# RchalYang/torchrl

Measured on AMD Instinct MI355X. Metric: env_steps_per_sec_ppo_2048env_halfcheetah_shape, higher is better.
Workload: dtype f32

## Files before the change

### torchrl_amd/csrc/k_ppo.hip

```cpp
#include <cstdlib>
#include "trl_common.h"
#include "trl_mlp.h"
#include "trl_head.h"
#include "trl_comm.h"

struct PpoDev {
  const float *obs, *acts, *advs, *rets, *old_values, *old_logp;
  const int64_t* row_idx;
  int rows_mb, N;
  const double* adv_raw;
  double n_global;
  const float *pf_params, *vf_params;
  float clip_para, entropy_coeff;
  int clipped_value_loss, tanh_action;
  int loss_mode;
  float* partial;
  double* scal_partial;
  int n_wg, n_pf, p_stride;
  int D, A;
};

template <int D, int H, int A> struct PpoShape {
  static_assert(H == 64 && D > 16 && D <= 32 && A <= 8, "instantiated for 16 < D <= 32, H == 64, A <= 8");
  static constexpr int P_PF = MlpFlat<D, H, A>::P_PF, P_VF = MlpFlat<D, H, 1>::P_VF;
  static constexpr int P_STRIDE = ((P_PF > P_VF ? P_PF : P_VF) + 63) & ~63;
};

#define WV_WAVES 4
#ifdef TRL_EXP_CLK
#define WCLK_DECL long long clk_prev = clock64(); float clk_acc[24]; for (int q_ = 0; q_ < 24; ++q_) clk_acc[q_] = 0.f;
#define WCLK(ph) { __builtin_amdgcn_sched_barrier(0); const long long c_ = clock64(); clk_acc[ph] += (float)(c_ - clk_prev); clk_prev = c_; __builtin_amdgcn_sched_barrier(0); }
#else
#define WCLK_DECL
#define WCLK(ph)
#endif
#define WV_THREADS (64 * WV_WAVES)
#define LDT 20
#define LDW 68

template <int D, int H, int A> struct WvShape {
  static_assert(H == 64 && (D == 17 || D == 32) && A <= 8, "instantiated for D == 17 / 32, H == 64, A <= 8");
  static constexpr int O_W2F = 0, O_W2B = H * LDW, O_B1 = 2 * H * LDW, O_B2 = O_B1 + H, O_SCR = O_B2 + H;
  static constexpr int O_H1 = 0, O_H2 = H * LDT, O_DZ2 = 2 * H * LDT, O_DO = 3 * H * LDT, WSCR = O_DO + 16 * LDT;
  static constexpr int P_STRIDE = PpoShape<D, H, A>::P_STRIDE;
  static constexpr int MAIN = O_SCR + WV_WAVES * WSCR, FOLD = WV_WAVES * P_STRIDE;
  static constexpr int LDS_FLOATS = MAIN > FOLD ? MAIN : FOLD;
};

template <int D, int H, int A> struct WvShapeSD : WvShape<D, H, A> {
  using B = WvShape<D, H, A>;
  static constexpr int P_PF_SD = H * D + H + H * H + H + 2 * A * H + 2 * A, P_VF = MlpFlat<D, H, 1>::P_VF;
  static constexpr int P_STRIDE = ((P_PF_SD > P_VF ? P_PF_SD : P_VF) + 63) & ~63;
  static constexpr int FOLD = WV_WAVES * P_STRIDE;
  static constexpr int LDS_FLOATS = B::MAIN > FOLD ? B::MAIN : FOLD;
};
template <int D, int H, int A, int HEAD> struct WvPick { using T = WvShape<D, H, A>; };
template <int D, int H, int A> struct WvPick<D, H, A, HEAD_SD> { using T = WvShapeSD<D, H, A>; };
#define SD_HALF_LOG_2PI_PLUS_HALF 1.4189385332046727f

__device__ __forceinline__ f32x4 lds4(const float* p) { return *reinterpret_cast<const f32x4*>(p); }
__device__ __forceinline__ float row_sum16(float v) {
  v += __builtin_bit_cast(float, __builtin_amdgcn_update_dpp(0, __builtin_bit_cast(int, v), 0x128, 0xF, 0xF, false));
  v += __builtin_bit_cast(float, __builtin_amdgcn_update_dpp(0, __builtin_bit_cast(int, v), 0x124, 0xF, 0xF, false));
  v += __builtin_bit_cast(float, __builtin_amdgcn_update_dpp(0, __builtin_bit_cast(int, v), 0x122, 0xF, 0xF, false));
  v += __builtin_bit_cast(float, __builtin_amdgcn_update_dpp(0, __builtin_bit_cast(int, v), 0x121, 0xF, 0xF, false));
  return v;
}

template <int D, int H, int A, int ACT, bool IS_PF, bool CONTIG, bool RT, int HEAD = HEAD_GAUSS>
__device__ void ppo_wave_pass(const PpoDev& a, float* lds, int wg_in_net, int n_wg_net) {
  using S = typename WvPick<D, H, A, HEAD>::T;
  constexpr bool WIDE = D > 17,
                 CAT = HEAD == HEAD_CAT, SD = HEAD == HEAD_SD,
                 SDP = SD && IS_PF;
  static_assert(!WIDE || RT, "the wide tile exists as a runtime-dims instantiation only");
  static_assert(!CAT || (IS_PF && RT), "the categorical head is a policy pass of the runtime-dims kernels");
  static_assert(!SD || RT, "the state-dependent-std head belongs to the runtime-dims kernels");
  constexpr int AS = CAT ? 1 : 0;
  const int Dr = RT ? a.D : D;
  const int O = IS_PF ? (RT ? a.A : A) : 1;
  const int OH = SDP ? 2 * O : O;
  const int F_W1 = 0, F_B1 = H * Dr, F_W2 = F_B1 + H, F_B2 = F_W2 + H * H, F_W3 = F_B2 + H, F_B3 = F_W3 + OH * H,
            F_LS = F_B3 + OH, F_END = (CAT || SDP) ? F_LS : F_LS + O;
  auto sd_has = [&](int o) -> bool { return (o & 7) < O; };
  auto sd_row = [&](int o) -> int { return o < 8 ? o : O + (o - 8); };
  const int PS = RT ? a.p_stride : S::P_STRIDE;
  const int tid = threadIdx.x, lane = tid & 63, wave = tid >> 6;
  const int j = lane & 15, g = lane >> 4, i = j;
  const float* gp = IS_PF ? a.pf_params : a.vf_params;
  WCLK_DECL
  float* W2F = lds + S::O_W2F;
  float* W2B = lds + S::O_W2B;
  float* scr = lds + S::O_SCR + wave * S::WSCR;
  float* H1S = scr + S::O_H1;
  float* H2S = scr + S::O_H2;
  float* DZ2S = scr + S::O_DZ2;
  float* DOS = scr + S::O_DO;

  const double adv_s1 = IS_PF ? a.adv_raw[0] : 0.0, adv_s2 = IS_PF ? a.adv_raw[1] : 0.0;
  const int B = a.rows_mb * a.N;
  const int n_tiles = (B + 15) / 16;
  const int tile_stride = n_wg_net * WV_WAVES;

  float xq[5], xtq[4], lq[6];
  float xq2[4], xtq2[4];
  int tile = wg_in_net * WV_WAVES + wave;
  const int tpr = a.N >> 4;
  int p1r = 0, p1c = 0, p2r = 0, p2c = 0, st_r = 0, st_c = 0;
  int64_t ridx1 = 0, ridx2 = 0;
  bool fv[4], fv2[4];
  const bool f16 = !WIDE && (!RT || Dr > 16), jv = !RT || i < Dr, jv2 = WIDE && 16 + i < Dr;
  const unsigned ox16 = (unsigned)(j * Dr + (f16 ? 16 : 0)) * 4u, os = (unsigned)j * 4u;
  unsigned oxq[4], oxt[4], oa_[4], oxq2[4], oxt2[4];
#pragma unroll
  for (int q = 0; q < 4; ++q) {
    fv[q] = !RT || 4 * g + q < Dr;
    fv2[q] = WIDE && 16 + 4 * g + q < Dr;
    oxq[q] = (unsigned)(j * Dr + (fv[q] ? 4 * g + q : 0)) * 4u;
    oxt[q] = (unsigned)((4 * g + q) * Dr + (jv ? i : 0)) * 4u;
    oxq2[q] = (unsigned)(j * Dr + (fv2[q] ? 16 + 4 * g + q : 0)) * 4u;
    oxt2[q] = (unsigned)((4 * g + q) * Dr + (jv2 ? 16 + i : 0)) * 4u;
    if constexpr (SDP) oa_[q] = (unsigned)(j * O + (4 * (g & 1) + q < O ? 4 * (g & 1) + q : 0)) * 4u;
    else oa_[q] = CAT ? (unsigned)j * 4u : (unsigned)(j * O + (4 * g + q < O ? 4 * g + q : 0)) * 4u;
  }
  auto ldb = [](const float* base, unsigned byte_off) -> float {
    return *reinterpret_cast<const float*>(reinterpret_cast<const char*>(base) + byte_off);
  };
  auto pos_advance = [&](int& r, int& c) { c += st_c; r += st_r; if (c >= tpr) { c -= tpr; ++r; } };
  auto load_ridx = [&](int r) -> int64_t {
    const int rr = r < a.rows_mb ? r : 0;
    return a.row_idx ? a.row_idx[rr] : (int64_t)rr;
  };
  auto fetch_contig = [&](int64_t ridx, int r, int c) {
    const int64_t cell0 = (r < a.rows_mb) ? ridx * a.N + 16 * c : 0;
    const float* ob = a.obs + cell0 * Dr;
#pragma unroll
    for (int q = 0; q < 4; ++q) xq[q] = ldb(ob, oxq[q]);
// ... 66 lines not shown
      fetch_inputs(pn, nt * 16);
      fetch_row(nt + tile_stride);
    }
  };
  if constexpr (CONTIG) {
    const int t0 = __builtin_amdgcn_readfirstlane(tile);
    const int ts = __builtin_amdgcn_readfirstlane(tile_stride);
    st_r = ts / tpr; st_c = ts - st_r * tpr;
    int r0 = t0 / tpr, c0 = t0 - (t0 / tpr) * tpr;
    fetch_contig(load_ridx(r0), r0, c0);
    p1r = r0; p1c = c0;
    pos_advance(p1r, p1c);
    ridx1 = load_ridx(p1r);
    p2r = p1r; p2c = p1c;
    pos_advance(p2r, p2c);
    ridx2 = load_ridx(p2r);
  } else {
    fetch_row(tile);
    const int64_t p0 = (tile * 16 + j < B) ? ridx_nn * a.N + e_nn : 0;
    fetch_inputs(p0, tile * 16);
    fetch_row(tile + tile_stride);
  }
  constexpr int NV = H * H / (4 * WV_THREADS);
  f32x4 wv[NV], wt[NV];
  const int tc = tid & 63, tq = tid >> 6;
  const float bias1 = tid < H ? gp[F_B1 + tid] : 0.0f, bias2 = tid < H ? gp[F_B2 + tid] : 0.0f;
  {
    static_assert(WV_THREADS == 256 && H == 64, "the transposed staging maps (column, 4 rows) onto 256 threads");
    const bool w2_al = !RT || ((reinterpret_cast<uintptr_t>(gp + F_W2) & 15) == 0);
#pragma unroll
    for (int t = 0; t < NV; ++t) {
      if (w2_al) wv[t] = *reinterpret_cast<const f32x4*>(gp + F_W2 + 4 * (tid + WV_THREADS * t));
      else {
#pragma unroll
        for (int x = 0; x < 4; ++x) wv[t][x] = gp[F_W2 + 4 * (tid + WV_THREADS * t) + x];
      }
    }
#pragma unroll
    for (int t = 0; t < NV; ++t)
#pragma unroll
      for (int x = 0; x < 4; ++x) wt[t][x] = gp[F_W2 + (4 * (tq + 4 * t) + x) * H + tc];
  }
  for (int e = lane; e < 16 * LDT; e += 64) DOS[e] = 0.0f;
  float w1[4][5], w3h[4][4], w3t[4][4];
  float w1b[4][4];
#pragma unroll
  for (int so = 0; so < 4; ++so) {
    const int row = 16 * so + i;
#pragma unroll
    for (int r = 0; r < 4; ++r) w1[so][r] = fv[r] ? gp[F_W1 + row * Dr + (fv[r] ? 4 * g + r : 0)] : 0.0f;
    w1[so][4] = (g == 0 && f16) ? gp[F_W1 + row * Dr + (f16 ? 16 : 0)] : 0.0f;
    if constexpr (WIDE) {
#pragma unroll
      for (int r = 0; r < 4; ++r) w1b[so][r] = fv2[r] ? gp[F_W1 + row * Dr + (fv2[r] ? 16 + 4 * g + r : 0)] : 0.0f;
    }
#pragma unroll
    for (int r = 0; r < 4; ++r) {
      if constexpr (SDP) {
        const int o = 4 * g + r;
        w3h[so][r] = sd_has(i) ? gp[F_W3 + (sd_has(i) ? sd_row(i) : 0) * H + 16 * so + 4 * g + r] : 0.0f;
        w3t[so][r] = sd_has(o) ? gp[F_W3 + (sd_has(o) ? sd_row(o) : 0) * H + row] : 0.0f;
      } else if constexpr (IS_PF) {
        w3h[so][r] = (i < O) ? gp[F_W3 + (i < O ? i : 0) * H + 16 * so + 4 * g + r] : 0.0f;
        const int o = 4 * g + r;
        w3t[so][r] = (o < O) ? gp[F_W3 + (o < O ? o : 0) * H + row] : 0.0f;
      } else {
        w3h[so][r] = gp[F_W3 + 16 * so + 4 * g + r];
        w3t[so][r] = 0.0f;
      }
    }
  }
  float lsv[4], ivv[4], b3v[4], lspass[4];
#pragma unroll
  for (int r = 0; r < 4; ++r) {
    const int o = 4 * g + r;
    const float raw = (IS_PF && !CAT && !SDP && o < O) ? gp[F_LS + (o < O ? o : 0)] : 0.0f;
    lsv[r] = fminf(fmaxf(raw, -20.0f), 2.0f);
    ivv[r] = __expf(-2.0f * lsv[r]);
    lspass[r] = (raw >= -20.0f && raw <= 2.0f) ? 1.0f : 0.0f;
    if constexpr (SDP) b3v[r] = sd_has(o) ? gp[F_B3 + (sd_has(o) ? sd_row(o) : 0)] : 0.0f;
    else b3v[r] = (o < O) ? gp[F_B3 + (o < O ? o : 0)] : 0.0f;
  }
  const float vb3 = IS_PF ? 0.0f : gp[F_B3];
#pragma unroll
  for (int t = 0; t < NV; ++t) {
    const int e = 4 * (tid + WV_THREADS * t), r = e / H, c = e - r * H;
    *reinterpret_cast<f32x4*>(W2F + r * LDW + c) = wv[t];
    *reinterpret_cast<f32x4*>(W2B + tc * LDW + 4 * (tq + 4 * t)) = wt[t];
  }
  if (tid < H) { lds[S::O_B1 + tid] = bias1; lds[S::O_B2 + tid] = bias2; }
  __syncthreads();

  const double ng = a.n_global;
  const double adv_mean = adv_s1 / ng;
  const double adv_var = (adv_s2 - adv_s1 * adv_s1 / ng) / (ng - 1.0);
  const float adv_mu = (float)adv_mean;
  const float adv_rstd = 1.0f / ((float)sqrt(fmax(adv_var, 0.0)) + 1e-5f);
  const float inv_b = (float)(1.0 / ng);

  f32x4 gW2[4][4], gW1[4], gW3[4];
  f32x4 gW1b[4];
  float gb1[4][4], gb2[4][4], gW1c[4][4];
  float db3[4], dls[4], stv[7];
  float ent_sum = 0.0f;
  float sdst[8] = {0.0f, 0.0f, -INFINITY, -INFINITY, 0.0f, 0.0f, -INFINITY, -INFINITY}, sd_cnt = 0.0f;
#pragma unroll
  for (int x = 0; x < 4; ++x) {
    gW1[x] = gW3[x] = gW1b[x] = f32x4{0.f, 0.f, 0.f, 0.f};
    db3[x] = dls[x] = 0.0f;
#pragma unroll
    for (int y = 0; y < 4; ++y) { gW2[x][y] = f32x4{0.f, 0.f, 0.f, 0.f}; gb1[x][y] = gb2[x][y] = gW1c[x][y] = 0.0f; }
  }
#pragma unroll
  for (int k = 0; k < 7; ++k) stv[k] = (k >= 2 && k <= 5) ? -INFINITY : 0.0f;

  WCLK(0)
  for (; tile < n_tiles; tile += tile_stride) {
    const int s = tile * 16 + j;
    const bool valid = CONTIG ? true : (s < B);
    float xb[5], xt[4], lin[6], xb2[4], xt2[4];
#pragma unroll
    for (int r = 0; r < 4; ++r) xb[r] = (valid && fv[r]) ? xq[r] : 0.0f;
    xb[4] = (valid && f16) ? xq[4] : 0.0f;
#pragma unroll
    for (int q = 0; q < 4; ++q) xt[q] = (jv && (CONTIG || tile * 16 + 4 * g + q < B)) ? xtq[q] : 0.0f;
    if constexpr (WIDE) {
#pragma unroll
      for (int q = 0; q < 4; ++q) {
        xb2[q] = (valid && fv2[q]) ? xq2[q] : 0.0f;
        xt2[q] = (jv2 && (CONTIG || tile * 16 + 4 * g + q < B)) ? xtq2[q] : 0.0f;
      }
    }
#pragma unroll
    for (int q = 0; q < 6; ++q) lin[q] = lq[q];
    const float x16 = xb[4];

#define PIN_DS() __builtin_amdgcn_sched_barrier(0x676)
    f32x4 h1[4], h2[4];
    f32x4 wq[4], bq;
#pragma unroll
    for (int so = 0; so < 4; ++so) h1[so] = lds4(lds + S::O_B1 + 16 * so + 4 * g);
#pragma unroll
    for (int sl = 0; sl < 4; ++sl) wq[sl] = lds4(W2F + i * LDW + 16 * sl + 4 * g);
    bq = lds4(lds + S::O_B2 + 4 * g);
    PIN_DS();
    WCLK(9)
#pragma unroll
    for (int q = 0; q < (WIDE ? 4 : 5); ++q)
#pragma unroll
      for (int so = 0; so < 4; ++so) h1[so] = mfma16(w1[so][q], xb[q], h1[so]);
    if constexpr (WIDE) {
#pragma unroll
      for (int q = 0; q < 4; ++q)
#pragma unroll
        for (int so = 0; so < 4; ++so) h1[so] = mfma16(w1b[so][q], xb2[q], h1[so]);
    }
    WCLK(10)
#pragma unroll
    for (int so = 0; so < 4; ++so)
#pragma unroll
      for (int r = 0; r < 4; ++r) {
        h1[so][r] = act_fn<ACT>(h1[so][r]);
        H1S[(16 * so + 4 * g + r) * LDT + j] = h1[so][r];
      }
    WCLK(1)
#pragma unroll
// ... 202 lines not shown
      }
#pragma unroll
      for (int so = 0; so < 4; ++so)
#pragma unroll
        for (int r = 0; r < 4; ++r) {
          dz2[so][r] = dv * w3h[so][r];
          gW3[so][r] = fmaf(dv, h2[so][r], gW3[so][r]);
        }
    }
#pragma unroll
    for (int so = 0; so < 4; ++so)
#pragma unroll
      for (int r = 0; r < 4; ++r) {
        dz2[so][r] *= act_grad<ACT>(h2[so][r]);
        gb2[so][r] += dz2[so][r];
        DZ2S[(16 * so + 4 * g + r) * LDT + j] = dz2[so][r];
      }

    WCLK(3)
    f32x4 dz1[4];
    f32x4 hb[4], za2;
#pragma unroll
    for (int so = 0; so < 4; ++so) dz1[so] = f32x4{0.f, 0.f, 0.f, 0.f};
#pragma unroll
    for (int sl = 0; sl < 4; ++sl) {
      f32x4 w[4];
#pragma unroll
      for (int so = 0; so < 4; ++so) w[so] = wb[so];
      if (sl < 3) {
#pragma unroll
        for (int so = 0; so < 4; ++so) wb[so] = lds4(W2B + (16 * so + i) * LDW + 16 * (sl + 1) + 4 * g);
      } else {
#pragma unroll
        for (int c = 0; c < 4; ++c) hb[c] = lds4(H1S + (16 * c + j) * LDT + 4 * g);
        za2 = lds4(DZ2S + i * LDT + 4 * g);
      }
      PIN_DS();
#pragma unroll
      for (int r = 0; r < 4; ++r)
#pragma unroll
        for (int so = 0; so < 4; ++so) dz1[so] = mfma16(w[so][r], dz2[sl][r], dz1[so]);
    }
    WCLK(17)
#pragma unroll
    for (int so = 0; so < 4; ++so)
#pragma unroll
      for (int r = 0; r < 4; ++r) {
        dz1[so][r] *= act_grad<ACT>(h1[so][r]);
        gb1[so][r] += dz1[so][r];
        if constexpr (!WIDE) gW1c[so][r] = fmaf(dz1[so][r], x16, gW1c[so][r]);
        H2S[(16 * so + 4 * g + r) * LDT + j] = dz1[so][r];
      }
    f32x4 za1[4];
#pragma unroll
    for (int so = 0; so < 4; ++so) za1[so] = lds4(H2S + (16 * so + i) * LDT + 4 * g);
    PIN_DS();

    WCLK(4)
#pragma unroll
    for (int so = 0; so < 4; ++so) {
      const f32x4 za = za2;
      if (so < 3) { za2 = lds4(DZ2S + (16 * (so + 1) + i) * LDT + 4 * g); PIN_DS(); }
#pragma unroll
      for (int q = 0; q < 4; ++q)
#pragma unroll
        for (int c = 0; c < 4; ++c) gW2[so][c] = mfma16(za[q], hb[c][q], gW2[so][c]);
    }
    WCLK(5)
#pragma unroll
    for (int so = 0; so < 4; ++so)
#pragma unroll
      for (int q = 0; q < 4; ++q) gW1[so] = mfma16(za1[so][q], xt[q], gW1[so]);
    if constexpr (WIDE) {
#pragma unroll
      for (int so = 0; so < 4; ++so)
#pragma unroll
        for (int q = 0; q < 4; ++q) gW1b[so] = mfma16(za1[so][q], xt2[q], gW1b[so]);
    }
#undef PIN_DS
    WCLK(6)
  }

  __syncthreads();
  float* gimg = lds + wave * S::P_STRIDE;
  for (int e = F_END + lane; e < PS; e += 64) gimg[e] = 0.0f;
#pragma unroll
  for (int so = 0; so < 4; ++so)
#pragma unroll
    for (int r = 0; r < 4; ++r) {
      const int f = 16 * so + 4 * g + r;
#pragma unroll
      for (int c = 0; c < 4; ++c) gimg[F_W2 + f * H + 16 * c + j] = gW2[so][c][r];
      if (jv) gimg[F_W1 + f * Dr + j] = gW1[so][r];
      if (WIDE && jv2) gimg[F_W1 + f * Dr + 16 + j] = gW1b[so][r];
      const float c16 = WIDE ? 0.0f : row_sum16(gW1c[so][r]), s1 = row_sum16(gb1[so][r]), s2 = row_sum16(gb2[so][r]);
      if (j == 0) { if (f16) gimg[F_W1 + f * Dr + 16] = c16; gimg[F_B1 + f] = s1; gimg[F_B2 + f] = s2; }
      if constexpr (IS_PF) {
        const int o = 4 * g + r;
        if constexpr (SDP) { if (sd_has(o)) gimg[F_W3 + sd_row(o) * H + 16 * so + j] = gW3[so][r]; }
        else if (o < O) gimg[F_W3 + o * H + 16 * so + j] = gW3[so][r];
      } else {
        const float w3s = row_sum16(gW3[so][r]);
        if (j == 0) gimg[F_W3 + f] = w3s;
      }
    }
#pragma unroll
  for (int r = 0; r < 4; ++r) {
    const int o = 4 * g + r;
    const float b3 = row_sum16(db3[r]), dl = row_sum16(dls[r]);
    if constexpr (SDP) { if (j == 0 && sd_has(o)) gimg[F_B3 + sd_row(o)] = b3; }
    else if (j == 0 && o < O) {
      gimg[F_B3 + o] = b3;
      if (IS_PF && !CAT) gimg[F_LS + o] = dl;
    }
  }
  WCLK(7)
  __syncthreads();
  const int wg = blockIdx.x;
  static_assert(S::P_STRIDE % 4 == 0, "partial rows are folded and stored 16 bytes at a time");
  for (int e4 = tid; e4 < PS / 4; e4 += WV_THREADS) {
    f32x4 acc = lds4(lds + 4 * e4);
#pragma unroll
    for (int w = 1; w < WV_WAVES; ++w) acc += lds4(lds + w * S::P_STRIDE + 4 * e4);
    *reinterpret_cast<f32x4*>(a.partial + (size_t)wg * a.p_stride + 4 * e4) = acc;
  }
  WCLK(8)
#ifdef TRL_EXP_CLK
  if (tid == 0) for (int ph = 0; ph < 24; ++ph) a.partial[(size_t)wg * a.p_stride + PS - 40 + ph] = clk_acc[ph];
#endif
  __syncthreads();
  double* sred = reinterpret_cast<double*>(lds);
  {
    const bool own = g == 0;
    const double v0 = wave_sum(own ? (double)stv[0] : 0.0), v1 = wave_sum(own ? (double)stv[1] : 0.0),
                 v6 = wave_sum(own ? (double)stv[6] : 0.0);
    const float v2 = wave_max(own ? stv[2] : -INFINITY), v3 = wave_max(own ? stv[3] : -INFINITY),
                v4 = wave_max(own ? stv[4] : -INFINITY), v5 = wave_max(own ? stv[5] : -INFINITY);
    double v7 = 0.0;
    if constexpr (CAT || SDP) v7 = wave_sum(own ? (double)ent_sum : 0.0);
    if (lane == 0) {
      double* p = sred + wave * 8;
      p[0] = v0; p[1] = v1; p[2] = v2; p[3] = v3; p[4] = v4; p[5] = v5; p[6] = v6; p[7] = v7;
    }
    if constexpr (SDP) {
      double e[SD_SCAL];
#pragma unroll
      for (int k = 0; k < 8; ++k) e[k] = (k & 2) ? (double)wave_max(sdst[k]) : wave_sum((double)sdst[k]);
      e[8] = wave_sum((double)sd_cnt);
      if (lane == 0) {
#pragma unroll
        for (int k = 0; k < SD_SCAL; ++k) sred[WV_WAVES * 8 + wave * SD_SCAL + k] = k < 9 ? e[k] : 0.0;
      }
    }
  }
  __syncthreads();
  if (tid < 8) {
    double r = sred[tid];
    for (int w = 1; w < WV_WAVES; ++w) {
      const double o = sred[w * 8 + tid];
      r = (tid >= 2 && tid <= 5) ? fmax(r, o) : r + o;
    }
    a.scal_partial[(size_t)wg * 8 + tid] = r;
  }
  if constexpr (SDP) {
    if (tid >= 64 && tid < 64 + SD_SCAL) {
      const int k = tid - 64;
      double r = sred[WV_WAVES * 8 + k];
      for (int w = 1; w < WV_WAVES; ++w) {
        const double o = sred[WV_WAVES * 8 + w * SD_SCAL + k];
        r = (k < 8 && (k & 2)) ? fmax(r, o) : r + o;
      }
      a.scal_partial[(size_t)a.n_wg * 8 + (size_t)wg * SD_SCAL + k] = r;
    }
  }
}

#define RED_CHUNK 64
#ifndef RED_WAVES
#define RED_WAVES 8
#endif
#ifndef RED_DEPTH
#define RED_DEPTH 16
#endif
__device__ __forceinline__ float fold_chain_tree(float (&acc)[RED_DEPTH]) {
#pragma unroll
  for (int st = RED_DEPTH / 2; st > 0; st >>= 1)
#pragma unroll
    for (int k = 0; k < st; ++k) acc[k] += acc[k + st];
  return acc[0];
}
__device__ __forceinline__ float fold_rows_wave(const float* __restrict__ src, int nrow, int p_stride, int w, bool in_range) {
  float acc[RED_DEPTH];
#pragma unroll
  for (int k = 0; k < RED_DEPTH; ++k) acc[k] = 0.0f;
  if (in_range) {
    for (; w < nrow; w += RED_DEPTH * RED_WAVES) {
      float v[RED_DEPTH];
#pragma unroll
      for (int k = 0; k < RED_DEPTH; ++k) v[k] = (w + RED_WAVES * k < nrow) ? src[(size_t)(w + RED_WAVES * k) * p_stride] : 0.0f;
#pragma unroll
      for (int k = 0; k < RED_DEPTH; ++k) acc[k] += v[k];
    }
  }
  return fold_chain_tree(acc);
}
__device__ __forceinline__ float fold_waves_tree(const float (*s_acc)[RED_CHUNK], int lane) {
  float t4[RED_WAVES / 4];
#pragma unroll
  for (int q = 0; q < RED_WAVES / 4; ++q)
    t4[q] = (s_acc[4 * q][lane] + s_acc[4 * q + 1][lane]) + (s_acc[4 * q + 2][lane] + s_acc[4 * q + 3][lane]);
// ... 319 lines not shown
      const float g_ = first ? gval0 : grads[ge];
      const float mo = first ? m_old : a.m[ge], vo = first ? v_old : a.v[ge], po = first ? p_old : a.params[ge];
      const float gr = g_ * a.grad_scale * s_coef[net];
      const float m = a.beta1 * mo + (1.0f - a.beta1) * gr;
      const float v = a.beta2 * vo + (1.0f - a.beta2) * gr * gr;
      a.m[ge] = m; a.v[ge] = v;
      const float denom = sqrtf(v) / bc2_sqrt + a.eps;
      a.params[ge] = po - ((net == 0 ? lr_pf : lr_vf) / bc1) * (m / denom);
    }
  }
}

template <int D, int H, int A, int ACT, bool CONTIG, bool RT, int HEAD = HEAD_GAUSS>
__global__ __launch_bounds__(WV_THREADS, 1) void ppo_grad_wave_kernel(PpoDev a) {
  static_assert(HEAD == HEAD_GAUSS || RT, "categorical / state-dependent-std head: runtime-dims tiles");
  constexpr int HEAD_VF = HEAD == HEAD_CAT ? HEAD_GAUSS : HEAD;
  extern __shared__ __attribute__((aligned(16))) float lds[];
#ifdef TRL_CHAIN_CLK
  const unsigned long long clk0 = wall_clock64();
#endif
  if ((int)blockIdx.x < a.n_pf) ppo_wave_pass<D, H, A, ACT, true, CONTIG, RT, HEAD>(a, lds, blockIdx.x, a.n_pf);
  else                          ppo_wave_pass<D, H, A, ACT, false, CONTIG, RT, HEAD_VF>(a, lds, blockIdx.x - a.n_pf, a.n_wg - a.n_pf);
#ifdef TRL_CHAIN_CLK
  __syncthreads();
  if (threadIdx.x == 0) {
    a.scal_partial[(size_t)blockIdx.x * 8 + 7] = (double)wall_clock64();
    float* pad = a.partial + (size_t)blockIdx.x * a.p_stride + a.p_stride - 3;
    pad[0] = (float)(clk0 >> 40); pad[1] = (float)((clk0 >> 20) & 0xFFFFFull); pad[2] = (float)(clk0 & 0xFFFFFull);
  }
#endif
}

template <int D, int H, int O, int ACT>
__global__ __launch_bounds__(256) void mlp2_forward_kernel(const float* __restrict__ params,
                                                           const float* __restrict__ x,
                                                           float* __restrict__ out, int M) {
  using L = MlpLds<D, H, O>;
  constexpr int NT = H / 32, KS = ksteps_for(D);
  __shared__ __attribute__((aligned(16))) float sp[L::SIZE];
  const int tid = threadIdx.x, lane = tid & 63, wave = tid >> 6, i = lane & 31, hi = lane >> 5;
  L::load(sp, params, false, tid, 256);
  __syncthreads();
  const int n_tiles = (M + 31) / 32;
  for (int tile = blockIdx.x * 4 + wave; tile < n_tiles; tile += gridDim.x * 4) {
    const int s = tile * 32 + i;
    float xb[KS];
#pragma unroll
    for (int q = 0; q < KS; ++q) { const int k = rowmap(q, hi); xb[q] = (k < D && s < M) ? x[(size_t)s * D + k] : 0.0f; }
    f32x16 h1[NT], h2[NT];
#pragma unroll
    for (int mo = 0; mo < NT; ++mo)
      h1[mo] = act_tile<ACT>(layer1_tile<D, L::LD1, KS>(bias_tile(sp + L::B1 + 32 * mo, hi), sp + L::W1, mo, xb, i, hi));
#pragma unroll
    for (int mo = 0; mo < NT; ++mo)
      h2[mo] = act_tile<ACT>(layer_tile<NT, L::LD2>(bias_tile(sp + L::B2 + 32 * mo, hi), sp + L::W2, mo, h1, i, hi));
    float o[O];
    head_fwd<NT, H, O>(sp + L::W3, sp + L::B3, h2, hi, o);
    if (hi == 0 && s < M) {
#pragma unroll
      for (int c = 0; c < O; ++c) out[(size_t)s * O + c] = o[c];
    }
  }
}

#define SHAPE_IS(d, h, o) (D == (d) && H == (h) && A == (o))

static int ppo_stride_for(int D, int H, int A, int head) {
  if (head == HEAD_GAUSS && SHAPE_IS(17, 64, 6)) return PpoShape<17, 64, 6>::P_STRIDE;
  if (head_shape_ok(head, D, H, A)) {
    const int p_pf = ppo_p_pf(D, H, A, head), p_vf = ppo_p_vf(D, H);
    return ((p_pf > p_vf ? p_pf : p_vf) + 63) & ~63;
  }
  trl_set_error("trl_ppo_%spartial_stride: shape D=%d H=%d A=%d not instantiated (H == 64, 2 <= D <= 32, %d <= A <= %d)",
                HEADS[head].tag, D, H, A, HEADS[head].a_min, HEADS[head].a_max);
  return TRL_EUNSUPPORTED;
}
extern "C" int trl_ppo_partial_stride(int D, int H, int A) { return ppo_stride_for(D, H, A, HEAD_GAUSS); }
extern "C" int trl_ppo_cat_partial_stride(int D, int H, int A) { return ppo_stride_for(D, H, A, HEAD_CAT); }
extern "C" int trl_ppo_sd_partial_stride(int D, int H, int A) { return ppo_stride_for(D, H, A, HEAD_SD); }
extern "C" int trl_ppo_cat_supported(int D, int H, int A, int act) { return head_supported(HEAD_CAT, D, H, A, act); }
extern "C" int trl_ppo_sd_supported(int D, int H, int A, int act) { return head_supported(HEAD_SD, D, H, A, act); }
extern "C" int trl_ppo_sd_scalar_stride(void) { return HEADS[HEAD_SD].scal_stride; }
static_assert(WvShapeSD<17, 64, 8>::P_STRIDE == 6400 && WvShapeSD<32, 64, 8>::P_STRIDE == 7360, "SD image strides at A = 8");
static_assert(WvShapeSD<32, 64, 8>::LDS_FLOATS * sizeof(float) <= 160 * 1024, "SD fold images fit the LDS");

template <int D, int H, int A, int ACT, bool CONTIG, bool RT, int HEAD>
static int launch_ppo_v(const PpoDev& d, hipStream_t s) {
  using S = typename WvPick<D, H, A, HEAD>::T;
  const size_t lds = S::LDS_FLOATS * sizeof(float);
  static bool attr_set = false;
  if (!attr_set) {
    hipError_t e = hipFuncSetAttribute((const void*)ppo_grad_wave_kernel<D, H, A, ACT, CONTIG, RT, HEAD>,
                                       hipFuncAttributeMaxDynamicSharedMemorySize, (int)lds);
    if (e != hipSuccess) { trl_set_error("ppo_grad: hipFuncSetAttribute: %s", hipGetErrorString(e)); return (int)e; }
    attr_set = true;
  }
  hipLaunchKernelGGL((ppo_grad_wave_kernel<D, H, A, ACT, CONTIG, RT, HEAD>), dim3(d.n_wg), dim3(WV_THREADS), lds, s, d);
  TRL_LAUNCH_CHECK();
  return TRL_OK;
}
template <int D, int H, int A, int ACT, bool RT, int HEAD = HEAD_GAUSS>
static int launch_ppo(const PpoDev& d, hipStream_t s) {
  return (d.N % 16 == 0) ? launch_ppo_v<D, H, A, ACT, true, RT, HEAD>(d, s) : launch_ppo_v<D, H, A, ACT, false, RT, HEAD>(d, s);
}

extern "C" int trl_ppo_wg_split(int D, int H, int A, int n_tiles, int n_wg) {
  if (n_wg < 2 || n_tiles <= 0) { trl_set_error("trl_ppo_wg_split: need n_wg >= 2 and n_tiles > 0"); return TRL_EINVAL; }
  const double c_pf = 16.7, c_vf = 12.1;
  int best = n_wg / 2;
  double best_t = 1e300;
  for (int x = 1; x < n_wg; ++x) {
    const double t_pf = (double)((n_tiles + WV_WAVES * x - 1) / (WV_WAVES * x)) * c_pf;
    const double t_vf = (double)((n_tiles + WV_WAVES * (n_wg - x) - 1) / (WV_WAVES * (n_wg - x))) * c_vf;
    const double t = t_pf > t_vf ? t_pf : t_vf;
    if (t < best_t - 1e-9 || (t < best_t + 1e-9 && abs(2 * x - n_wg) < abs(2 * best - n_wg))) { best_t = t; best = x; }
  }
  (void)D; (void)H; (void)A;
  return best;
}
static int resolve_pf_wgs(int n_wg, int n_wg_pf) { return n_wg_pf < 0 ? 0 : (n_wg_pf > 0 ? n_wg_pf : n_wg / 2); }

static int ppo_grad_launch(const trl_ppo_batch_t* p, void* stream, int head = HEAD_GAUSS) {
  if (!p) { trl_set_error("ppo_grad: null descriptor"); return TRL_EINVAL; }
  if (!head_supported(head, p->D, p->H, p->A, p->act)) {
    trl_set_error("ppo_%sgrad: shape D=%d H=%d A=%d act=%d not instantiated (H == 64, 2 <= D <= 32, %d <= A <= %d, Tanh / ReLU)",
                  HEADS[head].tag, p->D, p->H, p->A, p->act, HEADS[head].a_min, HEADS[head].a_max);
    return TRL_EUNSUPPORTED;
  }
  TRL_REQUIRE(p->obs && p->acts && p->advs && p->rets, "null rollout tensor");
  TRL_REQUIRE(p->loss_mode == TRL_LOSS_PPO_CLIP || p->loss_mode == TRL_LOSS_A2C, "unknown loss_mode");
  TRL_REQUIRE(p->loss_mode == TRL_LOSS_A2C || p->old_logp, "the clipped surrogate needs old_logp");
  TRL_REQUIRE(!p->clipped_value_loss || p->old_values, "the clipped value loss needs old_values");
  TRL_REQUIRE(p->adv_raw && (p->pf_params || p->vf_params) && p->partial && p->scal_partial, "null pointer");
  TRL_REQUIRE(p->rows_mb > 0 && p->N > 0, "empty minibatch");
  TRL_REQUIRE(p->n_wg >= 1 && (p->n_wg >= 2 || p->n_wg_pf == -1 || p->n_wg_pf == p->n_wg), "n_wg must be >= 2 (>= 1 for one network)");
  TRL_REQUIRE(p->n_wg_pf >= -1 && p->n_wg_pf <= p->n_wg, "n_wg_pf must be 0 (even split), in [1, n_wg], or -1 (value net only)");
  TRL_REQUIRE(p->n_wg_pf == p->n_wg || p->vf_params, "null value parameters");
  TRL_REQUIRE(p->n_wg_pf == -1 || p->pf_params, "null policy parameters");
  TRL_REQUIRE(p->n_global > 1.0, "n_global must exceed 1 (unbiased std)");
  const int D = p->D, H = p->H, A = p->A;
  TRL_REQUIRE(((uintptr_t)p->partial & 15) == 0 && (((uintptr_t)p->pf_params | (uintptr_t)p->vf_params) & 3) == 0,
              "partial rows must be 16-byte aligned, parameter blocks 4-byte aligned");
  TRL_REQUIRE(head != HEAD_GAUSS || !SHAPE_IS(17, 64, 6) || (((uintptr_t)p->pf_params | (uintptr_t)p->vf_params) & 15) == 0,
              "parameter blocks of the benchmark shape must be 16-byte aligned");
  PpoDev d;
  d.obs = p->obs; d.acts = p->acts; d.advs = p->advs; d.rets = p->rets; d.old_values = p->old_values;
  d.old_logp = p->old_logp; d.row_idx = p->row_idx; d.rows_mb = p->rows_mb; d.N = p->N;
  d.adv_raw = p->adv_raw; d.n_global = p->n_global; d.pf_params = p->pf_params; d.vf_params = p->vf_params;
  d.clip_para = p->clip_para; d.entropy_coeff = p->entropy_coeff;
  d.clipped_value_loss = p->clipped_value_loss; d.tanh_action = p->tanh_action; d.loss_mode = p->loss_mode;
  d.partial = p->partial; d.scal_partial = p->scal_partial; d.n_wg = p->n_wg;
  d.n_pf = resolve_pf_wgs(p->n_wg, p->n_wg_pf);
  d.D = D; d.A = A;
  hipStream_t s = (hipStream_t)stream;
  d.p_stride = ppo_stride_for(D, H, A, head);
  if (head == HEAD_CAT) d.tanh_action = 0;
  if (head == HEAD_GAUSS && SHAPE_IS(17, 64, 6))
    return p->act == TRL_ACT_TANH ? launch_ppo<17, 64, 6, TRL_ACT_TANH, false>(d, s) : launch_ppo<17, 64, 6, TRL_ACT_RELU, false>(d, s);
  return with_head(head, [&](auto hd) {
    return with_tile_act(D, p->act, [&](auto tile, auto act) {
      return launch_ppo<decltype(tile)::value, 64, 8, decltype(act)::value, true, decltype(hd)::value>(d, s);
    });
  });
}

extern "C" int trl_ppo_minibatch_grad_f32(const trl_ppo_batch_t* p, void* stream) { return ppo_grad_launch(p, stream); }
extern "C" int trl_ppo_cat_minibatch_grad_f32(const trl_ppo_batch_t* p, void* stream) { return ppo_grad_launch(p, stream, HEAD_CAT); }
// ... 397 lines not shown
```

Before: 98.21 million.

## Fold per-wave gradient tiles in MFMA register layout instead of scattered images

The cross-wave gradient reduction no longer scatters each wave's accumulators into a full parameter image in LDS. Instead, each wave writes its MFMA fragments as contiguous f32x4 tiles, and bias and column sums are reduced through a small transposed scratch rather than per-element DPP row sums. Each wave then folds one output slab across waves and writes the result directly to the global partial row. This is meant to cut LDS footprint, scattered scalar LDS stores and the separate fold pass, at the cost of more complex index mapping for scalar entries and uncoalesced scattered global stores.

```diff
diff --git a/torchrl_amd/csrc/k_ppo.hip b/torchrl_amd/csrc/k_ppo.hip
--- a/torchrl_amd/csrc/k_ppo.hip
+++ b/torchrl_amd/csrc/k_ppo.hip
@@ -43,16 +43,17 @@
   static constexpr int O_W2F = 0, O_W2B = H * LDW, O_B1 = 2 * H * LDW, O_B2 = O_B1 + H, O_SCR = O_B2 + H;
   static constexpr int O_H1 = 0, O_H2 = H * LDT, O_DZ2 = 2 * H * LDT, O_DO = 3 * H * LDT, WSCR = O_DO + 16 * LDT;
   static constexpr int P_STRIDE = PpoShape<D, H, A>::P_STRIDE;
-  static constexpr int MAIN = O_SCR + WV_WAVES * WSCR, FOLD = WV_WAVES * P_STRIDE;
-  static constexpr int LDS_FLOATS = MAIN > FOLD ? MAIN : FOLD;
+  static constexpr int MAIN = O_SCR + WV_WAVES * WSCR;
+  static constexpr int XS_W2 = 0, XS_W1 = 16, XS_W1B = 20, XS_W3 = D > 17 ? 24 : 20, XS_PF = XS_W3 + 4, XS_VF = XS_W3;
+  static constexpr int XSC_PF = 3 * H + 32, XSC_VF = 4 * H + 16;
+  static constexpr int XCH_PF = WV_WAVES * (XS_PF * 256 + XSC_PF), XCH_VF = WV_WAVES * (XS_VF * 256 + XSC_VF);
+  static constexpr int XCH = XCH_PF > XCH_VF ? XCH_PF : XCH_VF;
+  static constexpr int LDS_FLOATS = MAIN > XCH ? MAIN : XCH;
 };
 
 template <int D, int H, int A> struct WvShapeSD : WvShape<D, H, A> {
-  using B = WvShape<D, H, A>;
   static constexpr int P_PF_SD = H * D + H + H * H + H + 2 * A * H + 2 * A, P_VF = MlpFlat<D, H, 1>::P_VF;
   static constexpr int P_STRIDE = ((P_PF_SD > P_VF ? P_PF_SD : P_VF) + 63) & ~63;
-  static constexpr int FOLD = WV_WAVES * P_STRIDE;
-  static constexpr int LDS_FLOATS = B::MAIN > FOLD ? B::MAIN : FOLD;
 };
 template <int D, int H, int A, int HEAD> struct WvPick { using T = WvShape<D, H, A>; };
 template <int D, int H, int A> struct WvPick<D, H, A, HEAD_SD> { using T = WvShapeSD<D, H, A>; };
@@ -285,6 +286,11 @@
     else b3v[r] = (o < O) ? gp[F_B3 + (o < O ? o : 0)] : 0.0f;
   }
   const float vb3 = IS_PF ? 0.0f : gp[F_B3];
+#ifdef TRL_EXP_CLK
+  WCLK(22)
+  __builtin_amdgcn_s_waitcnt(0);
+  WCLK(23)
+#endif
 #pragma unroll
   for (int t = 0; t < NV; ++t) {
     const int e = 4 * (tid + WV_THREADS * t), r = e / H, c = e - r * H;
@@ -653,50 +659,106 @@
   }
 
   __syncthreads();
-  float* gimg = lds + wave * S::P_STRIDE;
-  for (int e = F_END + lane; e < PS; e += 64) gimg[e] = 0.0f;
-#pragma unroll
-  for (int so = 0; so < 4; ++so)
+  const int wg = blockIdx.x;
+  {
+    constexpr int NS = IS_PF ? S::XS_PF : S::XS_VF, SC = IS_PF ? S::XSC_PF : S::XSC_VF;
+    f32x4* xch = reinterpret_cast<f32x4*>(lds);
+    float* xsc = lds + WV_WAVES * NS * 256;
+    f32x4* xw = xch + (wave * NS) * 64 + lane;
+    float* sw = xsc + wave * SC;
+    {
+      constexpr int NK = IS_PF ? 3 : 4, TS = 17;
+      static_assert(NK * 16 <= 64 && NK * 16 * TS <= NS * 64, "one task per lane, inside the wave's own region");
+      f32x4* tr = xch + (wave * NS) * 64;
+#pragma unroll
+      for (int so = 0; so < 4; ++so) {
+        f32x4* te = tr + (4 * so + g) * TS + j;
+        te[0] = f32x4{gb1[so][0], gb1[so][1], gb1[so][2], gb1[so][3]};
+        te[16 * TS] = f32x4{gb2[so][0], gb2[so][1], gb2[so][2], gb2[so][3]};
+        te[32 * TS] = f32x4{gW1c[so][0], gW1c[so][1], gW1c[so][2], gW1c[so][3]};
+        if constexpr (!IS_PF) te[48 * TS] = gW3[so];
+      }
+      if (lane < NK * 16) {
+        const f32x4* x = tr + lane * TS;
+        const f32x4 even = ((x[0] + x[8]) + (x[4] + x[12])) + ((x[2] + x[10]) + (x[6] + x[14]));
+        const f32x4 odd = ((x[1] + x[9]) + (x[5] + x[13])) + ((x[3] + x[11]) + (x[7] + x[15]));
+        *reinterpret_cast<f32x4*>(sw + 4 * lane) = even + odd;
+      }
+    }
+#pragma unroll
+    for (int so = 0; so < 4; ++so) {
+#pragma unroll
+      for (int c = 0; c < 4; ++c) xw[(S::XS_W2 + 4 * so + c) * 64] = gW2[so][c];
+      xw[(S::XS_W1 + so) * 64] = gW1[so];
+      if constexpr (WIDE) xw[(S::XS_W1B + so) * 64] = gW1b[so];
+      if constexpr (IS_PF) xw[(S::XS_W3 + so) * 64] = gW3[so];
+    }
 #pragma unroll
     for (int r = 0; r < 4; ++r) {
-      const int f = 16 * so + 4 * g + r;
-#pragma unroll
-      for (int c = 0; c < 4; ++c) gimg[F_W2 + f * H + 16 * c + j] = gW2[so][c][r];
-      if (jv) gimg[F_W1 + f * Dr + j] = gW1[so][r];
-      if (WIDE && jv2) gimg[F_W1 + f * Dr + 16 + j] = gW1b[so][r];
-      const float c16 = WIDE ? 0.0f : row_sum16(gW1c[so][r]), s1 = row_sum16(gb1[so][r]), s2 = row_sum16(gb2[so][r]);
-      if (j == 0) { if (f16) gimg[F_W1 + f * Dr + 16] = c16; gimg[F_B1 + f] = s1; gimg[F_B2 + f] = s2; }
-      if constexpr (IS_PF) {
-        const int o = 4 * g + r;
-        if constexpr (SDP) { if (sd_has(o)) gimg[F_W3 + sd_row(o) * H + 16 * so + j] = gW3[so][r]; }
-        else if (o < O) gimg[F_W3 + o * H + 16 * so + j] = gW3[so][r];
+      const int o = 4 * g + r;
+      const float b3 = row_sum16(db3[r]), dl = row_sum16(dls[r]);
+      if (j == 0) {
+        if constexpr (IS_PF) { sw[3 * H + o] = b3; sw[3 * H + 16 + o] = dl; }
+        else sw[4 * H + o] = b3;
+      }
+    }
+    WCLK(7)
+    __syncthreads();
+    float* prow = a.partial + (size_t)wg * a.p_stride;
+    auto fold4 = [&](int slot) -> f32x4 {
+      const f32x4* p = xch + slot * 64 + lane;
+      f32x4 acc = p[0];
+#pragma unroll
+      for (int w = 1; w < WV_WAVES; ++w) acc += p[w * NS * 64];
+      return acc;
+    };
+    {
+      const int so = wave;
+      f32x4 t2[4];
+#pragma unroll
+      for (int c = 0; c < 4; ++c) t2[c] = fold4(S::XS_W2 + 4 * so + c);
+      const f32x4 t1 = fold4(S::XS_W1 + so);
+      f32x4 t1b = f32x4{0.f, 0.f, 0.f, 0.f}, t3 = f32x4{0.f, 0.f, 0.f, 0.f};
+      if constexpr (WIDE) t1b = fold4(S::XS_W1B + so);
+      if constexpr (IS_PF) t3 = fold4(S::XS_W3 + so);
+#pragma unroll
+      for (int r = 0; r < 4; ++r) {
+        const int f = 16 * so + 4 * g + r;
+#pragma unroll
+        for (int c = 0; c < 4; ++c) prow[F_W2 + f * H + 16 * c + j] = t2[c][r];
+        if (jv) prow[F_W1 + f * Dr + j] = t1[r];
+        if (WIDE && jv2) prow[F_W1 + f * Dr + 16 + j] = t1b[r];
+        if constexpr (IS_PF) {
+          const int o = 4 * g + r;
+          if constexpr (SDP) { if (sd_has(o)) prow[F_W3 + sd_row(o) * H + 16 * so + j] = t3[r]; }
+          else if (o < O) prow[F_W3 + o * H + 16 * so + j] = t3[r];
+        }
+      }
+    }
+    for (int k = tid; k < SC; k += WV_THREADS) {
+      float acc = xsc[k];
+#pragma unroll
+      for (int w = 1; w < WV_WAVES; ++w) acc += xsc[w * SC + k];
+      const int q = k & (H - 1);
+      int dst = -1;
+      if (k < H) dst = F_B1 + q;
+      else if (k < 2 * H) dst = F_B2 + q;
+      else if (k < 3 * H) { if (f16) dst = F_W1 + q * Dr + 16; }
+      else if constexpr (IS_PF) {
+        const int o = q & 15;
+        if (q < 16) { if constexpr (SDP) { if (sd_has(o)) dst = F_B3 + sd_row(o); } else if (o < O) dst = F_B3 + o; }
+        else if (!CAT && !SDP && o < O) dst = F_LS + o;
       } else {
-        const float w3s = row_sum16(gW3[so][r]);
-        if (j == 0) gimg[F_W3 + f] = w3s;
-      }
-    }
-#pragma unroll
-  for (int r = 0; r < 4; ++r) {
-    const int o = 4 * g + r;
-    const float b3 = row_sum16(db3[r]), dl = row_sum16(dls[r]);
-    if constexpr (SDP) { if (j == 0 && sd_has(o)) gimg[F_B3 + sd_row(o)] = b3; }
-    else if (j == 0 && o < O) {
-      gimg[F_B3 + o] = b3;
-      if (IS_PF && !CAT) gimg[F_LS + o] = dl;
-    }
-  }
-  WCLK(7)
-  __syncthreads();
-  const int wg = blockIdx.x;
-  static_assert(S::P_STRIDE % 4 == 0, "partial rows are folded and stored 16 bytes at a time");
-  for (int e4 = tid; e4 < PS / 4; e4 += WV_THREADS) {
-    f32x4 acc = lds4(lds + 4 * e4);
-#pragma unroll
-    for (int w = 1; w < WV_WAVES; ++w) acc += lds4(lds + w * S::P_STRIDE + 4 * e4);
-    *reinterpret_cast<f32x4*>(a.partial + (size_t)wg * a.p_stride + 4 * e4) = acc;
+        if (k < 4 * H) dst = F_W3 + q;
+        else if (q < O) dst = F_B3 + q;
+      }
+      if (dst >= 0) prow[dst] = acc;
+    }
+    for (int e = (IS_PF ? F_END : F_LS) + tid; e < PS; e += WV_THREADS) prow[e] = 0.0f;
   }
   WCLK(8)
 #ifdef TRL_EXP_CLK
+  __syncthreads();
   if (tid == 0) for (int ph = 0; ph < 24; ++ph) a.partial[(size_t)wg * a.p_stride + PS - 40 + ph] = clk_acc[ph];
 #endif
   __syncthreads();
@@ -1182,7 +1244,7 @@
 extern "C" int trl_ppo_sd_supported(int D, int H, int A, int act) { return head_supported(HEAD_SD, D, H, A, act); }
 extern "C" int trl_ppo_sd_scalar_stride(void) { return HEADS[HEAD_SD].scal_stride; }
 static_assert(WvShapeSD<17, 64, 8>::P_STRIDE == 6400 && WvShapeSD<32, 64, 8>::P_STRIDE == 7360, "SD image strides at A = 8");
-static_assert(WvShapeSD<32, 64, 8>::LDS_FLOATS * sizeof(float) <= 160 * 1024, "SD fold images fit the LDS");
+static_assert(WvShapeSD<32, 64, 8>::LDS_FLOATS * sizeof(float) <= 160 * 1024, "the wide tile's exchange area fits the LDS");
 
 template <int D, int H, int A, int ACT, bool CONTIG, bool RT, int HEAD>
 static int launch_ppo_v(const PpoDev& d, hipStream_t s) {
```

New measurement: 101.5 million, median of 6. 1.03x the previous value.
